# mederrata/spmf

Measured on NVIDIA B200. Metric: advi_elbo_grad_nnzK_per_s, higher is better.
Workload: dtype f32

## Files before the change

spmf_b200/csrc/spmf_hot_tile.cu:

```cuda
#include <cuda_bf16.h>
#include <cuda_runtime.h>
#include <stdint.h>
#include <stdlib.h>

#include "../../include/spmf_b200.h"
#include "spmf_record.cuh"
#include "spmf_umma_layout.cuh"
#include "spmf_umma_ptx.cuh"

namespace spmf {

__host__ __device__ __forceinline__ uint32_t core_off_g(int r, int kc, int cpr) {
  return (uint32_t)((((r >> 3) * cpr + kc) << 7) + ((r & 7) << 4));
}

template <int KP>
struct HotTile {
  static constexpr int KK = KP < 16 ? 16 : KP;
  static constexpr int CPR = KK / 8;
  static constexpr int ZCPR = CPR + 1;
  static constexpr int NZ = KK + 8;
  static constexpr int EV_TILE = 64 * KK * 2;
  static constexpr int EV_BLOCK = 2 * EV_TILE + 256;
  static constexpr int X_TILE = kTileABytes;
  static constexpr int STAGE = X_TILE + EV_BLOCK;
  static constexpr int Z_TILE = 128 * ZCPR * 16;
  static constexpr int ZCPR2 = 2 * ZCPR;
  static constexpr int W_TILE = 128 * 64 * 2;
  static constexpr bool WIDE = KK > 64;
  static constexpr bool MERGED = !WIDE;
  static constexpr int NSTAGE = WIDE ? 2 : 3;
  static constexpr int WBUF = WIDE ? 1 : 2;
  static constexpr int GHALF = WIDE ? 2 : 1;
  static constexpr int G_STRIDE = KK + 4;
  static constexpr int G_BYTES = (64 / GHALF) * G_STRIDE * 4;
  static constexpr int SMEM = NSTAGE * STAGE + 2 * Z_TILE + 2 * WBUF * W_TILE + G_BYTES + 128;
  static constexpr int ACC = MERGED ? 2 : 1;
  static constexpr int TM_S = 0, TM_DZ = 64, TM_GEV = 64 + ACC * KK, TM_GEV_STRIDE = ACC * NZ;
  static constexpr int TM_COLS = 512;
  static_assert(TM_GEV + 2 * TM_GEV_STRIDE <= 512, "tensor memory");
  static_assert(SMEM <= 227 * 1024, "shared memory");
};

__device__ __forceinline__ uint32_t pack_bf16(float a, float b) {
  __nv_bfloat162 v = __floats2bfloat162_rn(a, b);
  return *reinterpret_cast<uint32_t*>(&v);
}
__device__ __forceinline__ float bf16_lo(uint32_t p) { return __uint_as_float(p << 16); }
__device__ __forceinline__ float bf16_hi(uint32_t p) { return __uint_as_float(p & 0xffff0000u); }

template <int NC>
__device__ __forceinline__ void tmem_ld(uint32_t taddr, float* v) {
  static_assert(NC == 8 || NC == 16 || NC == 32, "tmem_ld width");
  uint32_t r[NC];
  if constexpr (NC == 32) {
    asm volatile(
        "tcgen05.ld.sync.aligned.32x32b.x32.b32 "
        "{%0, %1, %2, %3, %4, %5, %6, %7, %8, %9, %10, %11, %12, %13, %14, %15, "
        "%16, %17, %18, %19, %20, %21, %22, %23, %24, %25, %26, %27, %28, %29, %30, %31}, [%32];\n"
        : "=r"(r[0]), "=r"(r[1]), "=r"(r[2]), "=r"(r[3]), "=r"(r[4]), "=r"(r[5]), "=r"(r[6]), "=r"(r[7]),
          "=r"(r[8]), "=r"(r[9]), "=r"(r[10]), "=r"(r[11]), "=r"(r[12]), "=r"(r[13]), "=r"(r[14]), "=r"(r[15]),
          "=r"(r[16]), "=r"(r[17]), "=r"(r[18]), "=r"(r[19]), "=r"(r[20]), "=r"(r[21]), "=r"(r[22]), "=r"(r[23]),
          "=r"(r[24]), "=r"(r[25]), "=r"(r[26]), "=r"(r[27]), "=r"(r[28]), "=r"(r[29]), "=r"(r[30]), "=r"(r[31])
        : "r"(taddr));
  } else if constexpr (NC == 16) {
    asm volatile(
        "tcgen05.ld.sync.aligned.32x32b.x16.b32 "
        "{%0, %1, %2, %3, %4, %5, %6, %7, %8, %9, %10, %11, %12, %13, %14, %15}, [%16];\n"
        : "=r"(r[0]), "=r"(r[1]), "=r"(r[2]), "=r"(r[3]), "=r"(r[4]), "=r"(r[5]), "=r"(r[6]), "=r"(r[7]),
          "=r"(r[8]), "=r"(r[9]), "=r"(r[10]), "=r"(r[11]), "=r"(r[12]), "=r"(r[13]), "=r"(r[14]), "=r"(r[15])
        : "r"(taddr));
  } else {
    asm volatile("tcgen05.ld.sync.aligned.32x32b.x8.b32 {%0, %1, %2, %3, %4, %5, %6, %7}, [%8];\n"
                 : "=r"(r[0]), "=r"(r[1]), "=r"(r[2]), "=r"(r[3]), "=r"(r[4]), "=r"(r[5]), "=r"(r[6]), "=r"(r[7])
                 : "r"(taddr));
  }
  asm volatile("tcgen05.wait::ld.sync.aligned;" ::: "memory");
#pragma unroll
  for (int i = 0; i < NC; ++i) v[i] = __uint_as_float(r[i]);
}

__device__ __forceinline__ bool rate_ok_t(float lam) { return lam > 0.f && lam <= 3.402823466e38f; }

template <int KP, int SV>
__global__ void __launch_bounds__(256)
hot_ev_tiles_kernel(const float* __restrict__ EV, const float* __restrict__ PH, int D, int H,
                    unsigned char* __restrict__ EVt) {
  using T = HotTile<KP>;
  const int kc = blockIdx.x, s = blockIdx.y, nch = gridDim.x;
  const int q = s / SV, sv = s - q * SV;
  unsigned char* blk = EVt + ((size_t)s * nch + kc) * T::EV_BLOCK;
  for (int t = threadIdx.x; t < 64 * T::CPR; t += blockDim.x) {
    const int c = t / T::CPR, j = t - c * T::CPR;
    const int d = kc * 64 + c;
    float x[8];
#pragma unroll
    for (int h = 0; h < 2; ++h) {
      const int k = 8 * j + 4 * h;
      float4 v = make_float4(0.f, 0.f, 0.f, 0.f);
      if (d < H && k < KP)
        v = __ldg(reinterpret_cast<const float4*>(EV + ((size_t)q * D + d) * (SV * KP) + rec_pos(KP, SV, sv, k)));
      x[4 * h + 0] = v.x; x[4 * h + 1] = v.y; x[4 * h + 2] = v.z; x[4 * h + 3] = v.w;
    }
    uint32_t hi[4], lo[4];
#pragma unroll
    for (int p = 0; p < 4; ++p) {
      hi[p] = pack_bf16(x[2 * p], x[2 * p + 1]);
      lo[p] = pack_bf16(x[2 * p] - bf16_lo(hi[p]), x[2 * p + 1] - bf16_hi(hi[p]));
    }
    *reinterpret_cast<uint4*>(blk + core_off_g(c, j, 2 * T::CPR)) = make_uint4(hi[0], hi[1], hi[2], hi[3]);
    *reinterpret_cast<uint4*>(blk + core_off_g(c, T::CPR + j, 2 * T::CPR)) = make_uint4(lo[0], lo[1], lo[2], lo[3]);
    if (j == 0)
      reinterpret_cast<float*>(blk + 2 * T::EV_TILE)[c] = d < H ? __ldg(PH + ((size_t)q * D + d) * SV + sv) : 1.f;
  }
}

constexpr int kTileWorkThreads = 512;
constexpr int kTileThreads = kTileWorkThreads + 64;

template <int KP, int SV>
__global__ void __launch_bounds__(kTileThreads, 1)
hot_tile_kernel(const unsigned char* __restrict__ xhot, const unsigned char* __restrict__ EVt,
                const float* __restrict__ z, int nrows, int D, int H, int nch, int chunks_per_cta,
                float* __restrict__ dzacc, float* __restrict__ rowacc, float* __restrict__ GEV,
                float* __restrict__ Gphi, int* __restrict__ gflag) {
  using T = HotTile<KP>;
  constexpr int KK = T::KK, REC = SV * KP;
  extern __shared__ __align__(128) unsigned char smem_raw[];
  const uint32_t sbase = (smem_u32(smem_raw) + 127u) & ~127u;
  unsigned char* sp = smem_raw + (sbase - smem_u32(smem_raw));
  __shared__ __align__(8) unsigned long long mbar_store[T::NSTAGE + 3];
  __shared__ uint32_t tmem_slot;

  const int tid = threadIdx.x, warp = tid >> 5, lane = tid & 31;
  const int rt = tid & 127;
  const int hq = tid >> 7;
  const uint32_t lane_base = (uint32_t)((warp & 3) * 32) << 16;
  const int mt = blockIdx.x, s = blockIdx.y;
  const int q = s / SV, sv = s - q * SV;
  const int row = mt * 128 + rt;
  const int c_begin = blockIdx.z * chunks_per_cta;
  const int n = min(nch, c_begin + chunks_per_cta) - c_begin;
  if (n <= 0) return;

  const uint32_t sStage0 = sbase;
  const uint32_t sZ0 = sbase + (uint32_t)(T::NSTAGE * T::STAGE);
  const uint32_t sWb = sZ0 + 2u * (uint32_t)T::Z_TILE;
  unsigned char* const pZ0 = sp + T::NSTAGE * T::STAGE;
  unsigned char* const pWb = pZ0 + 2 * T::Z_TILE;

  uint32_t full[T::NSTAGE];
#pragma unroll
  for (int i = 0; i < T::NSTAGE; ++i) full[i] = smem_u32(&mbar_store[i]);
  const uint32_t bar_s = smem_u32(&mbar_store[T::NSTAGE]);
  const uint32_t bar_g[2] = {smem_u32(&mbar_store[T::NSTAGE + 1]), smem_u32(&mbar_store[T::NSTAGE + 2])};
  if (tid == 0) {
#pragma unroll
    for (int i = 0; i < T::NSTAGE; ++i) mbar_init(full[i], 1);
    mbar_init(bar_s, 1);
    mbar_init(bar_g[0], 2);
    mbar_init(bar_g[1], 2);
    asm volatile("fence.mbarrier_init.release.cluster;" ::: "memory");
  }
  if (warp == 3) {
    asm volatile("tcgen05.alloc.cta_group::1.sync.aligned.shared::cta.b32 [%0], %1;" ::"r"(smem_u32(&tmem_slot)),
                 "r"((uint32_t)T::TM_COLS)
                 : "memory");
    asm volatile("tcgen05.relinquish_alloc_permit.cta_group::1.sync.aligned;" ::: "memory");
  }

  const bool worker = tid < kTileWorkThreads;
  if (worker) {
    const float* zp = z + ((size_t)q * nrows + (row < nrows ? row : 0)) * REC;
#pragma unroll
    for (int j = 0; j < T::ZCPR; ++j) {
      if ((j & 3) != hq) continue;
      float zr[8];
#pragma unroll
      for (int e = 0; e < 8; ++e) zr[e] = 0.f;
      if (8 * j < KP && row < nrows) {
#pragma unroll
        for (int h = 0; h < 2; ++h) {
          if (8 * j + 4 * h < KP) {
            const float4 v = __ldg(reinterpret_cast<const float4*>(zp + rec_pos(KP, SV, sv, 8 * j + 4 * h)));
            zr[4 * h] = v.x; zr[4 * h + 1] = v.y; zr[4 * h + 2] = v.z; zr[4 * h + 3] = v.w;
          }
        }
      }
      if (8 * j == KK) zr[0] = 1.f;
      uint32_t hi[4], lo[4];
#pragma unroll
      for (int p = 0; p < 4; ++p) {
        const float a = zr[2 * p], b = zr[2 * p + 1];
        hi[p] = pack_bf16(a, b);
        lo[p] = pack_bf16(a - bf16_lo(hi[p]), b - bf16_hi(hi[p]));
      }
      *reinterpret_cast<uint4*>(pZ0 + core_off_g(rt, j, T::ZCPR2)) = make_uint4(hi[0], hi[1], hi[2], hi[3]);
      *reinterpret_cast<uint4*>(pZ0 + core_off_g(rt, T::ZCPR + j, T::ZCPR2)) = make_uint4(lo[0], lo[1], lo[2], lo[3]);
    }
  }
  asm volatile("fence.proxy.async.shared::cta;" ::: "memory");
  asm volatile("tcgen05.fence::before_thread_sync;" ::: "memory");
  __syncthreads();
  asm volatile("tcgen05.fence::after_thread_sync;" ::: "memory");
  const uint32_t tm = tmem_slot;

  const unsigned char* xsrc = xhot + ((size_t)mt * nch + c_begin) * T::X_TILE;
  const unsigned char* esrc = EVt + ((size_t)s * nch + c_begin) * T::EV_BLOCK;
  auto issue_load = [&](int i) {
    const int st = i % T::NSTAGE;
    const uint32_t dst = sStage0 + (uint32_t)(st * T::STAGE);
    mbar_expect_tx(full[st], (uint32_t)T::STAGE);
    tma_bulk_g2s(dst, xsrc + (size_t)i * T::X_TILE, T::X_TILE, full[st]);
    tma_bulk_g2s(dst + T::X_TILE, esrc + (size_t)i * T::EV_BLOCK, T::EV_BLOCK, full[st]);
  };
  auto wait_full = [&](int i) { mbar_wait(full[i % T::NSTAGE], (uint32_t)((i / T::NSTAGE) & 1)); };
  constexpr uint64_t kStageStep = (uint64_t)(T::STAGE >> 4);
  constexpr uint64_t kWStep = (uint64_t)((2 * T::W_TILE) >> 4);
  auto issue_p1 = [&](int i) {
    constexpr uint32_t ID = umma_idesc_bf16(128, 64, 0, 0);
    const uint64_t so = (uint64_t)(i % T::NSTAGE) * kStageStep;
    const uint64_t dZk[2] = {umma_desc(sZ0, 128, T::ZCPR2 * 128), umma_desc(sZ0 + T::ZCPR * 128, 128, T::ZCPR2 * 128)};
    const uint64_t dEk[2] = {umma_desc(sStage0 + T::X_TILE, 128, 2 * T::CPR * 128),
                             umma_desc(sStage0 + T::X_TILE + T::CPR * 128, 128, 2 * T::CPR * 128)};
#pragma unroll
    for (int t = 0; t < 3; ++t) {
      const uint64_t a = dZk[t == 2 ? 1 : 0], b = dEk[t == 1 ? 1 : 0] + so;
#pragma unroll
      for (int j = 0; j < KK / 16; ++j)
        umma_bf16_elect(tm + T::TM_S, a + (uint64_t)(j * 16), b + (uint64_t)(j * 16), ID, (t | j) ? 1u : 0u);
    }
    umma_commit_elect(bar_s);
  };
  float* const gst = reinterpret_cast<float*>(pWb + 2 * T::WBUF * T::W_TILE);
  auto flush_gev = [&](int i) {
    mbar_wait(bar_g[i & 1], (uint32_t)((i >> 1) & 1));
    asm volatile("tcgen05.fence::after_thread_sync;" ::: "memory");
    const uint32_t ta = tm + lane_base + T::TM_GEV + (uint32_t)((i & 1) * T::TM_GEV_STRIDE);
    const int m = (warp & 3) * 16 + lane;
    constexpr int NQD = KK >= 64 ? 4 : 2;
    constexpr int HK = KK / NQD;
    constexpr int ONES_Q = NQD == 4 ? 0 : 2;
    float g[HK], g1 = 0.f;
    if (hq < NQD) {
      tmem_ld<HK>(ta + HK * hq, g);
      if constexpr (T::MERGED) {
        float gb[HK];
        tmem_ld<HK>(ta + T::NZ + HK * hq, gb);
#pragma unroll
        for (int k = 0; k < HK; ++k) g[k] += gb[k];
      }
    }
    if (hq == ONES_Q) {
      float t8[8];
      tmem_ld<8>(ta + KK, t8);
      g1 = t8[0];
    }
    asm volatile("tcgen05.fence::before_thread_sync;" ::: "memory");
    constexpr int CPH = 64 / T::GHALF;
#pragma unroll
    for (int half = 0; half < T::GHALF; ++half) {
      if (half > 0) asm volatile("bar.sync 1, %0;" ::"n"(kTileWorkThreads) : "memory");
      const int ml = m - half * CPH;
      if (lane < 16 && ml >= 0 && ml < CPH) {
        if (hq < NQD) {
#pragma unroll
          for (int k = 0; k < HK; k += 4)
            *reinterpret_cast<float4*>(gst + ml * T::G_STRIDE + HK * hq + k) = make_float4(g[k], g[k + 1], g[k + 2], g[k + 3]);
        }
        if (hq == ONES_Q) gst[ml * T::G_STRIDE + KK] = g1;
      }
      asm volatile("bar.sync 1, %0;" ::"n"(kTileWorkThreads) : "memory");
      constexpr int TPC = KK / 4;
      constexpr int PASSES = (CPH * TPC + kTileWorkThreads - 1) / kTileWorkThreads;
#pragma unroll
      for (int ps = 0; ps < PASSES; ++ps) {
        const int idx = ps * kTileWorkThreads + tid;
        const int cl = idx / TPC, k = (idx % TPC) * 4;
        const int c = (c_begin + i) * 64 + half * CPH + cl;
        if (cl < CPH && c < H) {
          if (k < KP) {
            const float4 v = *reinterpret_cast<const float4*>(gst + cl * T::G_STRIDE + k);
            atomicAdd(reinterpret_cast<float4*>(GEV + ((size_t)q * D + c) * REC + rec_pos(KP, SV, sv, k)), v);
          }
          if ((idx % TPC) == TPC - 1) atomicAdd(Gphi + ((size_t)q * D + c) * SV + sv, gst[cl * T::G_STRIDE + KK]);
        }
      }
    }
  };

  if (warp == 17) {
    if (elect_one()) {
      issue_load(0);
      if (n > 1) issue_load(1);
      if (T::NSTAGE > 2 && n > 2) issue_load(2);
    }
    __syncwarp();
  }
  if (warp == 16) {
    wait_full(0);
    asm volatile("tcgen05.fence::after_thread_sync;" ::: "memory");
    issue_p1(0);
  }

  float xlog2 = 0.f, wmax = 0.f;
  for (int i = 0; i < n; ++i) {
    const int st = i % T::NSTAGE, wb = T::WBUF == 1 ? 0 : (i & 1), gb_ = i & 1;
    if (worker) {
    wait_full(i);
    mbar_wait(bar_s, (uint32_t)(i & 1));
    if (T::WBUF == 1 && i >= 1)
      mbar_wait(bar_g[(i - 1) & 1], (uint32_t)(((i - 1) >> 1) & 1));
    asm volatile("tcgen05.fence::after_thread_sync;" ::: "memory");

    {
      const unsigned char* xt = sp + st * T::STAGE;
      const float* ph = reinterpret_cast<const float*>(xt + T::X_TILE + 2 * T::EV_TILE) + 16 * hq;
      unsigned char* w0 = pWb + wb * 2 * T::W_TILE;
      float lam[16];
      tmem_ld<16>(tm + lane_base + T::TM_S + 16 * hq, lam);
#pragma unroll
      for (int j = 0; j < 2; ++j) {
        const uint32_t o = core_off(rt, 2 * hq + j);
        const uint4 xp = *reinterpret_cast<const uint4*>(xt + o);
        const uint32_t xw[4] = {xp.x, xp.y, xp.z, xp.w};
        const float4 p0 = *reinterpret_cast<const float4*>(ph + 8 * j);
        const float4 p1 = *reinterpret_cast<const float4*>(ph + 8 * j + 4);
        const float phv[8] = {p0.x, p0.y, p0.z, p0.w, p1.x, p1.y, p1.z, p1.w};
        float w[8];
#pragma unroll
        for (int e = 0; e < 8; ++e) {
          const float x = (e & 1) ? bf16_hi(xw[e >> 1]) : bf16_lo(xw[e >> 1]);
          const float l = fmaxf(lam[8 * j + e] + phv[e], 1e-30f);
          float lg, rc;
          asm("lg2.approx.ftz.f32 %0, %1;" : "=f"(lg) : "f"(l));
          asm("rcp.approx.ftz.f32 %0, %1;" : "=f"(rc) : "f"(l));
          w[e] = x * rc;
          wmax = fmaxf(wmax, w[e]);
          xlog2 = fmaf(x, lg, xlog2);
        }
        uint32_t hi[4], lo[4];
#pragma unroll
        for (int p = 0; p < 4; ++p) {
          hi[p] = pack_bf16(w[2 * p], w[2 * p + 1]);
          lo[p] = pack_bf16(w[2 * p] - bf16_lo(hi[p]), w[2 * p + 1] - bf16_hi(hi[p]));
        }
        *reinterpret_cast<uint4*>(w0 + o) = make_uint4(hi[0], hi[1], hi[2], hi[3]);
        *reinterpret_cast<uint4*>(w0 + T::W_TILE + o) = make_uint4(lo[0], lo[1], lo[2], lo[3]);
      }
    }
    }
    asm volatile("fence.proxy.async.shared::cta;" ::: "memory");
    asm volatile("tcgen05.fence::before_thread_sync;" ::: "memory");
    __syncthreads();

    if (warp == 17) {
      asm volatile("tcgen05.fence::after_thread_sync;" ::: "memory");
      const uint64_t wo = (uint64_t)wb * kWStep, so = (uint64_t)st * kStageStep;
      const uint64_t dWh = umma_desc(sWb, 128, 1024) + wo, dWl = umma_desc(sWb + T::W_TILE, 128, 1024) + wo;
      const uint64_t dEn = umma_desc(sStage0 + T::X_TILE, 2 * T::CPR * 128, 128) + so;
      constexpr uint64_t kEStep = (uint64_t)(2 * 2 * T::CPR * 128 / 16);
      if constexpr (T::MERGED) {
        constexpr uint32_t IDa = umma_idesc_bf16(128, 2 * KK, 0, 1), IDb = umma_idesc_bf16(128, KK, 0, 1);
#pragma unroll
        for (int j = 0; j < 4; ++j)
          umma_bf16_elect(tm + T::TM_DZ, dWh + (uint64_t)(j * 16), dEn + j * kEStep, IDa, (i | j) ? 1u : 0u);
#pragma unroll
        for (int j = 0; j < 4; ++j)
          umma_bf16_elect(tm + T::TM_DZ, dWl + (uint64_t)(j * 16), dEn + j * kEStep, IDb, 1u);
      } else {
        constexpr uint32_t ID = umma_idesc_bf16(128, KK, 0, 1);
        const uint64_t dEl = umma_desc(sStage0 + T::X_TILE + T::CPR * 128, 2 * T::CPR * 128, 128) + so;
#pragma unroll
        for (int j = 0; j < 4; ++j)
          umma_bf16_elect(tm + T::TM_DZ, dWh + (uint64_t)(j * 16), dEn + j * kEStep, ID, (i | j) ? 1u : 0u);
#pragma unroll
        for (int j = 0; j < 4; ++j)
          umma_bf16_elect(tm + T::TM_DZ, dWh + (uint64_t)(j * 16), dEl + j * kEStep, ID, 1u);
#pragma unroll
        for (int j = 0; j < 4; ++j)
          umma_bf16_elect(tm + T::TM_DZ, dWl + (uint64_t)(j * 16), dEn + j * kEStep, ID, 1u);
      }
      umma_commit_elect(bar_g[gb_]);
      if (i >= 1 && i + T::NSTAGE - 1 < n) {
        mbar_wait(bar_g[(i - 1) & 1], (uint32_t)(((i - 1) >> 1) & 1));
        if (elect_one()) issue_load(i + T::NSTAGE - 1);
        __syncwarp();
      }
    } else if (warp == 16) {
      asm volatile("tcgen05.fence::after_thread_sync;" ::: "memory");
      if (i + 1 < n) {
        wait_full(i + 1);
        asm volatile("tcgen05.fence::after_thread_sync;" ::: "memory");
        issue_p1(i + 1);
      }
      const uint64_t wo = (uint64_t)wb * kWStep;
      const uint64_t dWh = umma_desc(sWb, 1024, 128) + wo, dWl = umma_desc(sWb + T::W_TILE, 1024, 128) + wo;
      const uint64_t dZn = umma_desc(sZ0, T::ZCPR2 * 128, 128);
      constexpr uint64_t kZStep = (uint64_t)(2 * T::ZCPR2 * 128 / 16);
      const uint32_t tg = tm + T::TM_GEV + (uint32_t)(gb_ * T::TM_GEV_STRIDE);
      if constexpr (T::MERGED) {
        constexpr uint32_t IDa = umma_idesc_bf16(64, 2 * T::NZ, 1, 1), IDb = umma_idesc_bf16(64, T::NZ, 1, 1);
#pragma unroll
        for (int j = 0; j < 8; ++j)
          umma_bf16_elect(tg, dWh + (uint64_t)(j * (2048 / 16)), dZn + j * kZStep, IDa, j ? 1u : 0u);
#pragma unroll
        for (int j = 0; j < 8; ++j)
          umma_bf16_elect(tg, dWl + (uint64_t)(j * (2048 / 16)), dZn + j * kZStep, IDb, 1u);
      } else {
        constexpr uint32_t ID = umma_idesc_bf16(64, T::NZ, 1, 1);
        const uint64_t dZl = umma_desc(sZ0 + T::ZCPR * 128, T::ZCPR2 * 128, 128);
#pragma unroll
        for (int j = 0; j < 8; ++j)
          umma_bf16_elect(tg, dWh + (uint64_t)(j * (2048 / 16)), dZn + j * kZStep, ID, j ? 1u : 0u);
#pragma unroll
        for (int j = 0; j < 8; ++j)
          umma_bf16_elect(tg, dWh + (uint64_t)(j * (2048 / 16)), dZl + j * kZStep, ID, 1u);
#pragma unroll
        for (int j = 0; j < 8; ++j)
          umma_bf16_elect(tg, dWl + (uint64_t)(j * (2048 / 16)), dZn + j * kZStep, ID, 1u);
      }
      umma_commit_elect(bar_g[gb_]);
    } else if (i >= 1) {
      flush_gev(i - 1);
    }
  }
  if (worker) {
  asm volatile("bar.sync 1, %0;" ::"n"(kTileWorkThreads) : "memory");
  flush_gev(n - 1);

  {
    constexpr int QK = KK / 4;
    constexpr int LD = QK < 8 ? 8 : QK;
    float dzv[LD];
    const int col0 = QK >= 8 ? QK * hq : 8 * (hq >> 1);
    tmem_ld<LD>(tm + lane_base + T::TM_DZ + col0, dzv);
    if constexpr (T::MERGED) {
      float dzb[LD];
      tmem_ld<LD>(tm + lane_base + T::TM_DZ + KK + col0, dzb);
#pragma unroll
      for (int k = 0; k < LD; ++k) dzv[k] += dzb[k];
    }
    if (row < nrows) {
      float* dp = dzacc + ((size_t)q * nrows + row) * REC;
#pragma unroll
      for (int k = 0; k < QK; k += 4) {
        const int kk = QK * hq + k;
        const int src = (QK >= 8) ? k : 4 * (hq & 1) + k;
        if (kk < KP)
          atomicAdd(reinterpret_cast<float4*>(dp + rec_pos(KP, SV, sv, kk)),
                    make_float4(dzv[src], dzv[src + 1], dzv[src + 2], dzv[src + 3]));
      }
      atomicAdd(rowacc + ((size_t)q * nrows + row) * 4 * SV + sv, xlog2 * 0.6931471805599453f);
    }
    if (gflag && (!(wmax < 1e25f) || !(fabsf(xlog2) <= 3.402823466e38f))) atomicOr(gflag, 1);
  }
  }
  asm volatile("tcgen05.fence::before_thread_sync;" ::: "memory");
  __syncthreads();
  if (warp == 3) {
    asm volatile("tcgen05.dealloc.cta_group::1.sync.aligned.b32 %0, %1;" ::"r"(tm), "r"((uint32_t)T::TM_COLS) : "memory");
  }
}

template <int KP, int SV>
__global__ void __launch_bounds__(128)
rows_finish_kernel(const float* __restrict__ rowsum, const float* __restrict__ lgam, float inv_xi, int scale_rows,
                   int nrows, const double* __restrict__ vsum, const float* __restrict__ z,
                   float* __restrict__ dzr, float* __restrict__ rowacc, int* __restrict__ gflag) {
  constexpr int REC = SV * KP;
  static_assert(KP >= 4, "rows_finish: float4 k-vectors");
  constexpr int NCH = (REC + 127) / 128;
  const RecMap rm = rec_map(KP);
  const int row = blockIdx.x * 4 + (threadIdx.x >> 5), lane = threadIdx.x & 31, q = blockIdx.y;
  if (row >= nrows) return;
// ... 145 lines not shown
```

spmf_b200/csrc/spmf_umma.cu:

```cuda
#include <cuda_bf16.h>
#include <cuda_runtime.h>
#include <stdint.h>

#include "../../include/spmf_b200.h"
#include "spmf_umma_layout.cuh"
#include "spmf_umma_ptx.cuh"

namespace spmf {

constexpr int kGemmStages = 3;
constexpr int kGemmThreads = 128;

template <int N>
struct GemmSmem {
  static constexpr int A_BYTES = kTileABytes;
  static constexpr int B_BYTES = 3 * N * kGemmBK * 2;
  static constexpr int STAGE_BYTES = A_BYTES + B_BYTES;
  static constexpr int TOTAL = kGemmStages * STAGE_BYTES + 128;
};

template <int N>
__global__ void __launch_bounds__(kGemmThreads, 1)
umma_gemm3_kernel(const __nv_bfloat16* __restrict__ A, long long a_qstride, int M,
                  const __nv_bfloat16* __restrict__ B, long long b_qstride, float* __restrict__ C,
// ... 84 lines not shown

  const int row = m0 + tid;
  float* crow = C + (long long)row * ldc;
#pragma unroll
  for (int cb = 0; cb < N / 32; ++cb) {
    float v[32];
    tmem_ld32(tmem_acc + ((uint32_t)(warp * 32) << 16) + (uint32_t)(cb * 32), v);
    if (row < M) {
#pragma unroll
      for (int j = 0; j < 32; j += 4)
        atomicAdd(reinterpret_cast<float4*>(crow + cb * 32 + j), make_float4(v[j], v[j + 1], v[j + 2], v[j + 3]));
    }
  }
  asm volatile("tcgen05.fence::before_thread_sync;" ::: "memory");
  __syncthreads();
  if (warp == 2) {
    asm volatile("tcgen05.dealloc.cta_group::1.sync.aligned.b32 %0, %1;" ::"r"(tmem_acc), "r"((uint32_t)N) : "memory");
  }
}

__global__ void __launch_bounds__(256)
split3_transpose_kernel(const float* __restrict__ src, long long lds, long long src_qstride, int R, int Rpad,
                        int Ccols, __nv_bfloat16* __restrict__ dst, long long dst_qstride) {
  __shared__ float tile[32][33];
  const int q = blockIdx.z;
  src += (long long)q * src_qstride;
  dst += (long long)q * dst_qstride;
  const int r0 = blockIdx.x * 32, cbase = blockIdx.y * 32;
  const int tx = threadIdx.x & 31, ty = threadIdx.x >> 5;
#pragma unroll
  for (int i = 0; i < 4; ++i) {
    const int r = r0 + ty + 8 * i, c = cbase + tx;
    tile[ty + 8 * i][tx] = (r < R && c < Ccols) ? src[(long long)r * lds + c] : 0.f;
  }
  __syncthreads();
  const int c = cbase + (threadIdx.x >> 3), kq = (threadIdx.x & 7) * 4;
  if (c < Ccols && r0 + kq < Rpad) {
    __nv_bfloat16 o[3][4];
#pragma unroll
    for (int j = 0; j < 4; ++j) {
      const float x = tile[kq + j][threadIdx.x >> 3];
      const __nv_bfloat16 h = __float2bfloat16_rn(x);
      const float r1 = x - __bfloat162float(h);
      const __nv_bfloat16 m = __float2bfloat16_rn(r1);
      const float r2 = r1 - __bfloat162float(m);
      o[0][j] = h; o[1][j] = m; o[2][j] = __float2bfloat16_rn(r2);
    }
#pragma unroll
    for (int t = 0; t < 3; ++t)
      *reinterpret_cast<uint2*>(dst + tiledB_index(t, c, r0 + kq, Ccols)) = *reinterpret_cast<const uint2*>(o[t]);
  }
}

__global__ void __launch_bounds__(128, 1)
umma_probe_kernel(const unsigned char* __restrict__ a_img, int a_bytes, const unsigned char* __restrict__ b_img,
                  int b_bytes, int M, int N, int a_mn, int b_mn, int lbo_a, int sbo_a, int step_a, int lbo_b,
                  int sbo_b, int step_b, int nk, float* __restrict__ out) {
  extern __shared__ __align__(128) unsigned char smem_raw[];
  const uint32_t sbase = (smem_u32(smem_raw) + 127u) & ~127u;
  unsigned char* sp = smem_raw + (sbase - smem_u32(smem_raw));
  __shared__ __align__(8) unsigned long long mb;
  __shared__ uint32_t tslot;
  const int tid = threadIdx.x, warp = tid >> 5;
  const int a_pad = (a_bytes + 127) & ~127;
  for (int i = tid; i < a_bytes; i += 128) sp[i] = a_img[i];
  for (int i = tid; i < b_bytes; i += 128) sp[a_pad + i] = b_img[i];
  const uint32_t mbar = smem_u32(&mb);
  if (tid == 0) {
    mbar_init(mbar, 1);
    asm volatile("fence.mbarrier_init.release.cluster;" ::: "memory");
  }
  if (warp == 2) {
    asm volatile("tcgen05.alloc.cta_group::1.sync.aligned.shared::cta.b32 [%0], %1;" ::"r"(smem_u32(&tslot)), "r"(256u)
                 : "memory");
    asm volatile("tcgen05.relinquish_alloc_permit.cta_group::1.sync.aligned;" ::: "memory");
  }
  asm volatile("fence.proxy.async.shared::cta;" ::: "memory");
  asm volatile("tcgen05.fence::before_thread_sync;" ::: "memory");
  __syncthreads();
  asm volatile("tcgen05.fence::after_thread_sync;" ::: "memory");
  const uint32_t tacc = tslot;
  {
    const uint32_t taddr = tacc + ((uint32_t)(warp * 32) << 16);
    for (int c = 0; c < N; ++c)
      asm volatile("tcgen05.st.sync.aligned.32x32b.x1.b32 [%0], {%1};" ::"r"(taddr + c), "r"(0u) : "memory");
    asm volatile("tcgen05.wait::st.sync.aligned;" ::: "memory");
  }
  asm volatile("tcgen05.fence::before_thread_sync;" ::: "memory");
  __syncthreads();
  asm volatile("tcgen05.fence::after_thread_sync;" ::: "memory");
  if (tid == 0) {
    const uint32_t idesc = umma_idesc_bf16(M, N, a_mn, b_mn);
    for (int j = 0; j < nk; ++j) {
      const uint64_t ad = umma_desc(sbase + j * step_a, lbo_a, sbo_a);
      const uint64_t bd = umma_desc(sbase + a_pad + j * step_b, lbo_b, sbo_b);
      umma_bf16(tacc, ad, bd, idesc, j ? 1u : 0u);
    }
    umma_commit(mbar);
  }
  __syncwarp();
  mbar_wait(mbar, 0u);
  asm volatile("tcgen05.fence::after_thread_sync;" ::: "memory");
  for (int cb = 0; cb < N / 32; ++cb) {
    float v[32];
    tmem_ld32(tacc + ((uint32_t)(warp * 32) << 16) + (uint32_t)(cb * 32), v);
    for (int j = 0; j < 32; ++j) out[(long long)tid * N + cb * 32 + j] = v[j];
  }
  asm volatile("tcgen05.fence::before_thread_sync;" ::: "memory");
  __syncthreads();
  if (warp == 2) asm volatile("tcgen05.dealloc.cta_group::1.sync.aligned.b32 %0, %1;" ::"r"(tacc), "r"(256u) : "memory");
}

template <int N>
struct GemmAtSmem {
  static constexpr int A_BYTES = kTileABytes / 2;
  static constexpr int B_BYTES = 3 * N * kGemmBK * 2;
  static constexpr int STAGE_BYTES = A_BYTES + B_BYTES;
  static constexpr int TOTAL = kGemmStages * STAGE_BYTES + 128;
};

template <int N>
__global__ void __launch_bounds__(kGemmThreads, 1)
umma_gemm3_at_kernel(const __nv_bfloat16* __restrict__ X, int xchunks, int M,
                     const __nv_bfloat16* __restrict__ B, long long b_qstride, float* __restrict__ C,
                     long long ldc, long long c_qstride, int kchunks, int chunks_per_split, int nblocks) {
  using SM = GemmAtSmem<N>;
  extern __shared__ __align__(128) unsigned char smem_raw[];
  const uint32_t sbase = (smem_u32(smem_raw) + 127u) & ~127u;
  __shared__ __align__(8) unsigned long long mbar_store[2 * kGemmStages + 1];
  __shared__ uint32_t tmem_base_slot;

  const int tid = threadIdx.x, warp = tid >> 5, lane = tid & 31;
  const int kc = blockIdx.x;
  const int q = blockIdx.z / nblocks, nb = blockIdx.z - q * nblocks;
  const int c0 = blockIdx.y * chunks_per_split;
  const int c1 = min(kchunks, c0 + chunks_per_split);
  const int nchunks = c1 - c0;
  if (nchunks <= 0) return;
  B += (long long)q * b_qstride + (long long)nb * (N * kGemmBK);
  C += (long long)q * c_qstride + (long long)nb * N;
  const long long b_term = (long long)nblocks * N * kGemmBK;

  uint32_t full[kGemmStages], empty[kGemmStages];
#pragma unroll
  for (int i = 0; i < kGemmStages; ++i) {
    full[i] = smem_u32(&mbar_store[i]);
    empty[i] = smem_u32(&mbar_store[kGemmStages + i]);
  }
  const uint32_t done = smem_u32(&mbar_store[2 * kGemmStages]);
  if (tid == 0) {
#pragma unroll
    for (int i = 0; i < kGemmStages; ++i) { mbar_init(full[i], 1); mbar_init(empty[i], 1); }
    mbar_init(done, 1);
    asm volatile("fence.mbarrier_init.release.cluster;" ::: "memory");
  }
  if (warp == 2) {
    asm volatile("tcgen05.alloc.cta_group::1.sync.aligned.shared::cta.b32 [%0], %1;" ::"r"(smem_u32(&tmem_base_slot)),
                 "r"((uint32_t)N)
                 : "memory");
    asm volatile("tcgen05.relinquish_alloc_permit.cta_group::1.sync.aligned;" ::: "memory");
  }
  asm volatile("tcgen05.fence::before_thread_sync;" ::: "memory");
  __syncthreads();
// ... 125 lines not shown

extern "C" {

long long spmf_umma_tiled_a_elems(long long M, long long Kd) { return (M + 127) / 128 * 128 * ((Kd + 63) / 64 * 64); }
long long spmf_umma_tiled_b_elems(int N, long long Kd) { return 3LL * N * ((Kd + 63) / 64 * 64); }
long long spmf_umma_tiled_a_index(long long row, long long k, long long Kd) { return tiledA_index(row, k, Kd / kGemmBK); }

int spmf_umma_tile_a(const void* src, long long ld, int M, int Kd, void* dst, void* stream) {
  if (!src || !dst || M <= 0 || Kd <= 0 || Kd % kGemmBK) return SPMF_ERR_BAD_ARG;
  tile_a_kernel<<<148 * 4, 256, 0, (cudaStream_t)stream>>>((const __nv_bfloat16*)src, ld, M, Kd, (__nv_bfloat16*)dst);
  cudaError_t e = cudaGetLastError();
  return e == cudaSuccess ? SPMF_OK : (int)e;
}

int spmf_umma_gemm3(const void* A, long long a_qstride, int M, const void* B3, long long b_qstride, float* C,
                    long long ldc, long long c_qstride, int N, int Kd, int NQ, int splits, void* stream) {
  if (!A || !B3 || !C || M <= 0 || Kd <= 0 || NQ <= 0) return SPMF_ERR_BAD_ARG;
  if (Kd % kGemmBK || ldc % 4) return SPMF_ERR_BAD_ARG;
  if (((uintptr_t)A | (uintptr_t)B3 | (uintptr_t)C) & 15) return SPMF_ERR_BAD_ARG;
  cudaStream_t st = (cudaStream_t)stream;
  const __nv_bfloat16* a = (const __nv_bfloat16*)A;
  const __nv_bfloat16* b = (const __nv_bfloat16*)B3;
  switch (N) {
    case 32: return launch_gemm3<32>(a, a_qstride, M, b, b_qstride, C, ldc, c_qstride, Kd, NQ, splits, 1, st);
    case 64: return launch_gemm3<64>(a, a_qstride, M, b, b_qstride, C, ldc, c_qstride, Kd, NQ, splits, 1, st);
    case 128: case 256: case 512:
      return launch_gemm3<128>(a, a_qstride, M, b, b_qstride, C, ldc, c_qstride, Kd, NQ, splits, N / 128, st);
    default: return SPMF_ERR_UNSUPPORTED;
  }
}

int spmf_umma_gemm3_at(const void* X, int x_kd, int x_rows, int M, const void* B3, long long b_qstride, float* C,
                       long long ldc, long long c_qstride, int N, int NQ, int splits, void* stream) {
  if (!X || !B3 || !C || M <= 0 || x_kd <= 0 || x_rows <= 0 || NQ <= 0) return SPMF_ERR_BAD_ARG;
  if (x_kd % kGemmBK || M > x_kd || ldc % 4) return SPMF_ERR_BAD_ARG;
  if (((uintptr_t)X | (uintptr_t)B3 | (uintptr_t)C) & 15) return SPMF_ERR_BAD_ARG;
  const int Kd = (x_rows + 127) / 128 * 128;
  cudaStream_t st = (cudaStream_t)stream;
  const __nv_bfloat16* a = (const __nv_bfloat16*)X;
  const __nv_bfloat16* b = (const __nv_bfloat16*)B3;
  switch (N) {
    case 32: return launch_gemm3_at<32>(a, x_kd / kGemmBK, M, b, b_qstride, C, ldc, c_qstride, Kd, NQ, splits, 1, st);
    case 64: return launch_gemm3_at<64>(a, x_kd / kGemmBK, M, b, b_qstride, C, ldc, c_qstride, Kd, NQ, splits, 1, st);
    case 128: case 256: case 512:
      return launch_gemm3_at<128>(a, x_kd / kGemmBK, M, b, b_qstride, C, ldc, c_qstride, Kd, NQ, splits, N / 128, st);
    default: return SPMF_ERR_UNSUPPORTED;
  }
}

int spmf_umma_probe(const void* a_img, int a_bytes, const void* b_img, int b_bytes, int M, int N, int a_mn,
                    int b_mn, int lbo_a, int sbo_a, int step_a, int lbo_b, int sbo_b, int step_b, int nk,
                    float* out, void* stream) {
  if (!a_img || !b_img || !out || a_bytes <= 0 || b_bytes <= 0 || nk <= 0) return SPMF_ERR_BAD_ARG;
  if ((M != 64 && M != 128) || N % 32 || N < 32 || N > 256) return SPMF_ERR_BAD_ARG;
  const int smem = ((a_bytes + 127) & ~127) + b_bytes + 256;
  if (smem > 200 * 1024) return SPMF_ERR_BAD_ARG;
  cudaError_t e = cudaFuncSetAttribute(umma_probe_kernel, cudaFuncAttributeMaxDynamicSharedMemorySize, smem);
  if (e != cudaSuccess) return (int)e;
  umma_probe_kernel<<<1, 128, smem, (cudaStream_t)stream>>>((const unsigned char*)a_img, a_bytes,
                                                          (const unsigned char*)b_img, b_bytes, M, N, a_mn, b_mn,
                                                          lbo_a, sbo_a, step_a, lbo_b, sbo_b, step_b, nk, out);
  e = cudaGetLastError();
  return e == cudaSuccess ? SPMF_OK : (int)e;
}

int spmf_split3_transpose(const float* src, long long lds, long long src_qstride, int R, int Rpad, int Ccols,
                          void* dst3, long long dst_qstride, int NQ, void* stream) {
  if (!src || !dst3 || R <= 0 || Rpad < R || Rpad % kGemmBK || Ccols <= 0 || Ccols % 32 || NQ <= 0) return SPMF_ERR_BAD_ARG;
  dim3 grid((Rpad + 31) / 32, Ccols / 32, NQ);
  split3_transpose_kernel<<<grid, 256, 0, (cudaStream_t)stream>>>(src, lds, src_qstride, R, Rpad, Ccols,
                                                                  (__nv_bfloat16*)dst3, dst_qstride);
  cudaError_t e = cudaGetLastError();
  return e == cudaSuccess ? SPMF_OK : (int)e;
}

}
```

spmf_b200/csrc/spmf_umma_ptx.cuh:

```cuda
#pragma once
#include <cuda_runtime.h>
#include <stdint.h>

namespace spmf {

__device__ __forceinline__ uint32_t smem_u32(const void* p) {
  return (uint32_t)__cvta_generic_to_shared(p);
}

__device__ __forceinline__ uint64_t umma_desc(uint32_t saddr, uint32_t lbo, uint32_t sbo) {
  uint64_t d = 0;
  d |= (uint64_t)((saddr >> 4) & 0x3fffu);
  d |= (uint64_t)((lbo >> 4) & 0x3fffu) << 16;
  d |= (uint64_t)((sbo >> 4) & 0x3fffu) << 32;
  d |= (uint64_t)1 << 46;
  return d;
}

__host__ __device__ constexpr uint32_t umma_idesc_bf16(int M, int N, int a_mn = 0, int b_mn = 0) {
  return (1u << 4) | (1u << 7) | (1u << 10) | ((uint32_t)a_mn << 15) | ((uint32_t)b_mn << 16) |
         ((uint32_t)(N >> 3) << 17) | ((uint32_t)(M >> 4) << 24);
}

__device__ __forceinline__ void umma_bf16(uint32_t tmem_d, uint64_t adesc, uint64_t bdesc, uint32_t idesc,
                                          uint32_t accumulate) {
  asm volatile(
      "{\n\t"
      ".reg .pred p;\n\t"
      "setp.ne.b32 p, %4, 0;\n\t"
      "tcgen05.mma.cta_group::1.kind::f16 [%0], %1, %2, %3, p;\n\t"
      "}\n" ::"r"(tmem_d), "l"(adesc), "l"(bdesc), "r"(idesc), "r"(accumulate)
      : "memory");
}

__device__ __forceinline__ void umma_bf16_elect(uint32_t tmem_d, uint64_t adesc, uint64_t bdesc, uint32_t idesc,
                                                uint32_t accumulate) {
  asm volatile(
      "{\n\t"
      ".reg .pred p, e;\n\t"
      ".reg .b32 r;\n\t"
      "elect.sync r|e, 0xffffffff;\n\t"
      "setp.ne.b32 p, %4, 0;\n\t"
      "@e tcgen05.mma.cta_group::1.kind::f16 [%0], %1, %2, %3, p;\n\t"
      "}\n" ::"r"(tmem_d), "l"(adesc), "l"(bdesc), "r"(idesc), "r"(accumulate)
      : "memory");
}
__device__ __forceinline__ void umma_commit_elect(uint32_t mbar) {
  asm volatile(
      "{\n\t"
      ".reg .pred e;\n\t"
      ".reg .b32 r;\n\t"
      "elect.sync r|e, 0xffffffff;\n\t"
      "@e tcgen05.commit.cta_group::1.mbarrier::arrive::one.shared::cluster.b64 [%0];\n\t"
      "}\n" ::"r"(mbar)
      : "memory");
}
__device__ __forceinline__ bool elect_one() {
  uint32_t pred;
  asm volatile(
      "{\n\t"
      ".reg .pred e;\n\t"
      ".reg .b32 r;\n\t"
      "elect.sync r|e, 0xffffffff;\n\t"
      "selp.u32 %0, 1, 0, e;\n\t"
      "}\n"
      : "=r"(pred));
  return pred != 0;
}

__device__ __forceinline__ void umma_commit(uint32_t mbar) {
  asm volatile("tcgen05.commit.cta_group::1.mbarrier::arrive::one.shared::cluster.b64 [%0];" ::"r"(mbar)
               : "memory");
}

__device__ __forceinline__ void mbar_init(uint32_t mbar, uint32_t count) {
  asm volatile("mbarrier.init.shared::cta.b64 [%0], %1;" ::"r"(mbar), "r"(count) : "memory");
}

__device__ __forceinline__ void mbar_wait(uint32_t mbar, uint32_t parity) {
  uint32_t done;
  do {
    asm volatile(
        "{\n\t"
        ".reg .pred p;\n\t"
        "mbarrier.try_wait.parity.shared::cta.b64 p, [%1], %2;\n\t"
        "selp.u32 %0, 1, 0, p;\n\t"
        "}\n"
        : "=r"(done)
        : "r"(mbar), "r"(parity)
        : "memory");
  } while (!done);
}

__device__ __forceinline__ void tmem_ld32(uint32_t taddr, float (&v)[32]) {
  uint32_t r[32];
  asm volatile(
      "tcgen05.ld.sync.aligned.32x32b.x32.b32 "
      "{%0, %1, %2, %3, %4, %5, %6, %7, %8, %9, %10, %11, %12, %13, %14, %15, "
      "%16, %17, %18, %19, %20, %21, %22, %23, %24, %25, %26, %27, %28, %29, %30, %31}, [%32];\n"
      : "=r"(r[0]), "=r"(r[1]), "=r"(r[2]), "=r"(r[3]), "=r"(r[4]), "=r"(r[5]), "=r"(r[6]), "=r"(r[7]),
        "=r"(r[8]), "=r"(r[9]), "=r"(r[10]), "=r"(r[11]), "=r"(r[12]), "=r"(r[13]), "=r"(r[14]), "=r"(r[15]),
        "=r"(r[16]), "=r"(r[17]), "=r"(r[18]), "=r"(r[19]), "=r"(r[20]), "=r"(r[21]), "=r"(r[22]), "=r"(r[23]),
        "=r"(r[24]), "=r"(r[25]), "=r"(r[26]), "=r"(r[27]), "=r"(r[28]), "=r"(r[29]), "=r"(r[30]), "=r"(r[31])
      : "r"(taddr));
  asm volatile("tcgen05.wait::ld.sync.aligned;" ::: "memory");
#pragma unroll
  for (int i = 0; i < 32; ++i) v[i] = __uint_as_float(r[i]);
}

__device__ __forceinline__ void mbar_expect_tx(uint32_t mbar, uint32_t bytes) {
  asm volatile("mbarrier.arrive.expect_tx.shared::cta.b64 _, [%0], %1;" ::"r"(mbar), "r"(bytes) : "memory");
}
__device__ __forceinline__ void tma_bulk_g2s(uint32_t dst, const void* src, uint32_t bytes, uint32_t mbar) {
  asm volatile("cp.async.bulk.shared::cluster.global.mbarrier::complete_tx::bytes [%0], [%1], %2, [%3];" ::"r"(dst),
               "l"(src), "r"(bytes), "r"(mbar)
               : "memory");
}

}
```

Measured before the change: 255.1 billion.

## Feed UMMA A operands from tensor memory and double-buffer P1 scores for small K

For K up to 32, the z and W bf16 hi/lo tiles are also written into tensor memory, and the P1 and P2 MMAs read their A operand from TMEM instead of shared-memory descriptors. The P1 score accumulator gets a second TMEM buffer with its own mbarrier, so the MMA warp can issue P1 for chunk i+2 while workers process chunk i. The load pipeline also deepens to four stages. This aims to cut shared-memory operand traffic and the P1-to-worker serialization, at the cost of extra tcgen05.st stores and waits in the worker threads. The probe kernel gains a TMEM-A test mode.

```diff
diff --git a/spmf_b200/csrc/spmf_hot_tile.cu b/spmf_b200/csrc/spmf_hot_tile.cu
--- a/spmf_b200/csrc/spmf_hot_tile.cu
+++ b/spmf_b200/csrc/spmf_hot_tile.cu
@@ -29,7 +29,9 @@
   static constexpr int W_TILE = 128 * 64 * 2;
   static constexpr bool WIDE = KK > 64;
   static constexpr bool MERGED = !WIDE;
-  static constexpr int NSTAGE = WIDE ? 2 : 3;
+  static constexpr bool TMEM_A = KK <= 32;
+  static constexpr int SBUF = TMEM_A ? 2 : 1;
+  static constexpr int NSTAGE = WIDE ? 2 : (SBUF == 2 ? 4 : 3);
   static constexpr int WBUF = WIDE ? 1 : 2;
   static constexpr int GHALF = WIDE ? 2 : 1;
   static constexpr int G_STRIDE = KK + 4;
@@ -38,7 +40,11 @@
   static constexpr int ACC = MERGED ? 2 : 1;
   static constexpr int TM_S = 0, TM_DZ = 64, TM_GEV = 64 + ACC * KK, TM_GEV_STRIDE = ACC * NZ;
   static constexpr int TM_COLS = 512;
-  static_assert(TM_GEV + 2 * TM_GEV_STRIDE <= 512, "tensor memory");
+  static constexpr int TM_S1 = TM_GEV + 2 * TM_GEV_STRIDE;
+  static constexpr int TM_W_STRIDE = 64, TM_W = TM_COLS - 2 * TM_W_STRIDE, TM_Z = TM_W - KK;
+  static constexpr int TM_USED = TM_S1 + (TMEM_A ? 64 + KK + 2 * TM_W_STRIDE : 0);
+  static_assert(TM_USED <= TM_COLS && (!TMEM_A || TM_S1 + 64 <= TM_Z), "tensor memory");
+  static_assert(!TMEM_A || MERGED, "tensor-memory A operands: merged-term P2 only");
   static_assert(SMEM <= 227 * 1024, "shared memory");
 };
 
@@ -129,7 +135,7 @@
   extern __shared__ __align__(128) unsigned char smem_raw[];
   const uint32_t sbase = (smem_u32(smem_raw) + 127u) & ~127u;
   unsigned char* sp = smem_raw + (sbase - smem_u32(smem_raw));
-  __shared__ __align__(8) unsigned long long mbar_store[T::NSTAGE + 3];
+  __shared__ __align__(8) unsigned long long mbar_store[T::NSTAGE + 2 + T::SBUF];
   __shared__ uint32_t tmem_slot;
 
   const int tid = threadIdx.x, warp = tid >> 5, lane = tid & 31;
@@ -152,12 +158,15 @@
   uint32_t full[T::NSTAGE];
 #pragma unroll
   for (int i = 0; i < T::NSTAGE; ++i) full[i] = smem_u32(&mbar_store[i]);
-  const uint32_t bar_s = smem_u32(&mbar_store[T::NSTAGE]);
-  const uint32_t bar_g[2] = {smem_u32(&mbar_store[T::NSTAGE + 1]), smem_u32(&mbar_store[T::NSTAGE + 2])};
+  const uint32_t bar_g[2] = {smem_u32(&mbar_store[T::NSTAGE]), smem_u32(&mbar_store[T::NSTAGE + 1])};
+  uint32_t bar_s[T::SBUF];
+#pragma unroll
+  for (int b = 0; b < T::SBUF; ++b) bar_s[b] = smem_u32(&mbar_store[T::NSTAGE + 2 + b]);
   if (tid == 0) {
 #pragma unroll
     for (int i = 0; i < T::NSTAGE; ++i) mbar_init(full[i], 1);
-    mbar_init(bar_s, 1);
+#pragma unroll
+    for (int b = 0; b < T::SBUF; ++b) mbar_init(bar_s[b], 1);
     mbar_init(bar_g[0], 2);
     mbar_init(bar_g[1], 2);
     asm volatile("fence.mbarrier_init.release.cluster;" ::: "memory");
@@ -169,6 +178,11 @@
     asm volatile("tcgen05.relinquish_alloc_permit.cta_group::1.sync.aligned;" ::: "memory");
   }
 
+  asm volatile("tcgen05.fence::before_thread_sync;" ::: "memory");
+  __syncthreads();
+  asm volatile("tcgen05.fence::after_thread_sync;" ::: "memory");
+  const uint32_t tm = tmem_slot;
+
   const bool worker = tid < kTileWorkThreads;
   if (worker) {
     const float* zp = z + ((size_t)q * nrows + (row < nrows ? row : 0)) * REC;
@@ -197,13 +211,19 @@
       }
       *reinterpret_cast<uint4*>(pZ0 + core_off_g(rt, j, T::ZCPR2)) = make_uint4(hi[0], hi[1], hi[2], hi[3]);
       *reinterpret_cast<uint4*>(pZ0 + core_off_g(rt, T::ZCPR + j, T::ZCPR2)) = make_uint4(lo[0], lo[1], lo[2], lo[3]);
-    }
+      if constexpr (T::TMEM_A) {
+        if (j < T::CPR) {
+          tmem_st_x4(tm + lane_base + T::TM_Z + 4 * j, make_uint4(hi[0], hi[1], hi[2], hi[3]));
+          tmem_st_x4(tm + lane_base + T::TM_Z + KK / 2 + 4 * j, make_uint4(lo[0], lo[1], lo[2], lo[3]));
+        }
+      }
+    }
+    if constexpr (T::TMEM_A) tmem_st_wait();
   }
   asm volatile("fence.proxy.async.shared::cta;" ::: "memory");
   asm volatile("tcgen05.fence::before_thread_sync;" ::: "memory");
   __syncthreads();
   asm volatile("tcgen05.fence::after_thread_sync;" ::: "memory");
-  const uint32_t tm = tmem_slot;
 
   const unsigned char* xsrc = xhot + ((size_t)mt * nch + c_begin) * T::X_TILE;
   const unsigned char* esrc = EVt + ((size_t)s * nch + c_begin) * T::EV_BLOCK;
@@ -219,18 +239,25 @@
   constexpr uint64_t kWStep = (uint64_t)((2 * T::W_TILE) >> 4);
   auto issue_p1 = [&](int i) {
     constexpr uint32_t ID = umma_idesc_bf16(128, 64, 0, 0);
+    const uint32_t ts = tm + ((i & 1) && T::SBUF == 2 ? T::TM_S1 : T::TM_S);
     const uint64_t so = (uint64_t)(i % T::NSTAGE) * kStageStep;
     const uint64_t dZk[2] = {umma_desc(sZ0, 128, T::ZCPR2 * 128), umma_desc(sZ0 + T::ZCPR * 128, 128, T::ZCPR2 * 128)};
     const uint64_t dEk[2] = {umma_desc(sStage0 + T::X_TILE, 128, 2 * T::CPR * 128),
                              umma_desc(sStage0 + T::X_TILE + T::CPR * 128, 128, 2 * T::CPR * 128)};
 #pragma unroll
     for (int t = 0; t < 3; ++t) {
-      const uint64_t a = dZk[t == 2 ? 1 : 0], b = dEk[t == 1 ? 1 : 0] + so;
-#pragma unroll
-      for (int j = 0; j < KK / 16; ++j)
-        umma_bf16_elect(tm + T::TM_S, a + (uint64_t)(j * 16), b + (uint64_t)(j * 16), ID, (t | j) ? 1u : 0u);
-    }
-    umma_commit_elect(bar_s);
+      const uint64_t b = dEk[t == 1 ? 1 : 0] + so;
+#pragma unroll
+      for (int j = 0; j < KK / 16; ++j) {
+        if constexpr (T::TMEM_A)
+          umma_bf16_tmem_a_elect(ts, tm + T::TM_Z + (t == 2 ? KK / 2 : 0) + 8 * j, b + (uint64_t)(j * 16), ID,
+                                 (t | j) ? 1u : 0u);
+        else
+          umma_bf16_elect(ts, dZk[t == 2 ? 1 : 0] + (uint64_t)(j * 16), b + (uint64_t)(j * 16), ID,
+                          (t | j) ? 1u : 0u);
+      }
+    }
+    umma_commit_elect(bar_s[(i & 1) % T::SBUF]);
   };
   float* const gst = reinterpret_cast<float*>(pWb + 2 * T::WBUF * T::W_TILE);
   auto flush_gev = [&](int i) {
@@ -291,16 +318,21 @@
 
   if (warp == 17) {
     if (elect_one()) {
-      issue_load(0);
-      if (n > 1) issue_load(1);
-      if (T::NSTAGE > 2 && n > 2) issue_load(2);
+#pragma unroll
+      for (int k = 0; k < T::NSTAGE; ++k)
+        if (k < n) issue_load(k);
     }
     __syncwarp();
   }
   if (warp == 16) {
-    wait_full(0);
-    asm volatile("tcgen05.fence::after_thread_sync;" ::: "memory");
-    issue_p1(0);
+#pragma unroll
+    for (int k = 0; k < T::SBUF; ++k) {
+      if (k < n) {
+        wait_full(k);
+        asm volatile("tcgen05.fence::after_thread_sync;" ::: "memory");
+        issue_p1(k);
+      }
+    }
   }
 
   float xlog2 = 0.f, wmax = 0.f;
@@ -308,7 +340,7 @@
     const int st = i % T::NSTAGE, wb = T::WBUF == 1 ? 0 : (i & 1), gb_ = i & 1;
     if (worker) {
     wait_full(i);
-    mbar_wait(bar_s, (uint32_t)(i & 1));
+    mbar_wait(bar_s[(i & 1) % T::SBUF], (uint32_t)((i / T::SBUF) & 1));
     if (T::WBUF == 1 && i >= 1)
       mbar_wait(bar_g[(i - 1) & 1], (uint32_t)(((i - 1) >> 1) & 1));
     asm volatile("tcgen05.fence::after_thread_sync;" ::: "memory");
@@ -318,7 +350,7 @@
       const float* ph = reinterpret_cast<const float*>(xt + T::X_TILE + 2 * T::EV_TILE) + 16 * hq;
       unsigned char* w0 = pWb + wb * 2 * T::W_TILE;
       float lam[16];
-      tmem_ld<16>(tm + lane_base + T::TM_S + 16 * hq, lam);
+      tmem_ld<16>(tm + lane_base + ((i & 1) && T::SBUF == 2 ? T::TM_S1 : T::TM_S) + 16 * hq, lam);
 #pragma unroll
       for (int j = 0; j < 2; ++j) {
         const uint32_t o = core_off(rt, 2 * hq + j);
@@ -347,7 +379,13 @@
         }
         *reinterpret_cast<uint4*>(w0 + o) = make_uint4(hi[0], hi[1], hi[2], hi[3]);
         *reinterpret_cast<uint4*>(w0 + T::W_TILE + o) = make_uint4(lo[0], lo[1], lo[2], lo[3]);
-      }
+        if constexpr (T::TMEM_A) {
+          const uint32_t tw = tm + lane_base + T::TM_W + (uint32_t)(wb * T::TM_W_STRIDE) + 8 * hq + 4 * j;
+          tmem_st_x4(tw, make_uint4(hi[0], hi[1], hi[2], hi[3]));
+          tmem_st_x4(tw + 32, make_uint4(lo[0], lo[1], lo[2], lo[3]));
+        }
+      }
+      if constexpr (T::TMEM_A) tmem_st_wait();
     }
     }
     asm volatile("fence.proxy.async.shared::cta;" ::: "memory");
@@ -362,12 +400,21 @@
       constexpr uint64_t kEStep = (uint64_t)(2 * 2 * T::CPR * 128 / 16);
       if constexpr (T::MERGED) {
         constexpr uint32_t IDa = umma_idesc_bf16(128, 2 * KK, 0, 1), IDb = umma_idesc_bf16(128, KK, 0, 1);
-#pragma unroll
-        for (int j = 0; j < 4; ++j)
-          umma_bf16_elect(tm + T::TM_DZ, dWh + (uint64_t)(j * 16), dEn + j * kEStep, IDa, (i | j) ? 1u : 0u);
-#pragma unroll
-        for (int j = 0; j < 4; ++j)
-          umma_bf16_elect(tm + T::TM_DZ, dWl + (uint64_t)(j * 16), dEn + j * kEStep, IDb, 1u);
+        const uint32_t tWh = tm + T::TM_W + (uint32_t)(wb * T::TM_W_STRIDE), tWl = tWh + 32;
+#pragma unroll
+        for (int j = 0; j < 4; ++j) {
+          if constexpr (T::TMEM_A)
+            umma_bf16_tmem_a_elect(tm + T::TM_DZ, tWh + 8 * j, dEn + j * kEStep, IDa, (i | j) ? 1u : 0u);
+          else
+            umma_bf16_elect(tm + T::TM_DZ, dWh + (uint64_t)(j * 16), dEn + j * kEStep, IDa, (i | j) ? 1u : 0u);
+        }
+#pragma unroll
+        for (int j = 0; j < 4; ++j) {
+          if constexpr (T::TMEM_A)
+            umma_bf16_tmem_a_elect(tm + T::TM_DZ, tWl + 8 * j, dEn + j * kEStep, IDb, 1u);
+          else
+            umma_bf16_elect(tm + T::TM_DZ, dWl + (uint64_t)(j * 16), dEn + j * kEStep, IDb, 1u);
+        }
       } else {
         constexpr uint32_t ID = umma_idesc_bf16(128, KK, 0, 1);
         const uint64_t dEl = umma_desc(sStage0 + T::X_TILE + T::CPR * 128, 2 * T::CPR * 128, 128) + so;
@@ -389,7 +436,7 @@
       }
     } else if (warp == 16) {
       asm volatile("tcgen05.fence::after_thread_sync;" ::: "memory");
-      if (i + 1 < n) {
+      if (T::SBUF == 1 && i + 1 < n) {
         wait_full(i + 1);
         asm volatile("tcgen05.fence::after_thread_sync;" ::: "memory");
         issue_p1(i + 1);
@@ -421,6 +468,11 @@
           umma_bf16_elect(tg, dWl + (uint64_t)(j * (2048 / 16)), dZn + j * kZStep, ID, 1u);
       }
       umma_commit_elect(bar_g[gb_]);
+      if (T::SBUF == 2 && i + 2 < n) {
+        wait_full(i + 2);
+        asm volatile("tcgen05.fence::after_thread_sync;" ::: "memory");
+        issue_p1(i + 2);
+      }
     } else if (i >= 1) {
       flush_gev(i - 1);
     }
diff --git a/spmf_b200/csrc/spmf_umma.cu b/spmf_b200/csrc/spmf_umma.cu
--- a/spmf_b200/csrc/spmf_umma.cu
+++ b/spmf_b200/csrc/spmf_umma.cu
@@ -160,6 +160,7 @@
   }
 }
 
+constexpr int kProbeTmemA = 256;
 __global__ void __launch_bounds__(128, 1)
 umma_probe_kernel(const unsigned char* __restrict__ a_img, int a_bytes, const unsigned char* __restrict__ b_img,
                   int b_bytes, int M, int N, int a_mn, int b_mn, int lbo_a, int sbo_a, int step_a, int lbo_b,
@@ -170,8 +171,10 @@
   __shared__ __align__(8) unsigned long long mb;
   __shared__ uint32_t tslot;
   const int tid = threadIdx.x, warp = tid >> 5;
-  const int a_pad = (a_bytes + 127) & ~127;
-  for (int i = tid; i < a_bytes; i += 128) sp[i] = a_img[i];
+  const bool a_tmem = a_mn == 2;
+  const int a_pad = a_tmem ? 0 : (a_bytes + 127) & ~127;
+  if (!a_tmem)
+    for (int i = tid; i < a_bytes; i += 128) sp[i] = a_img[i];
   for (int i = tid; i < b_bytes; i += 128) sp[a_pad + i] = b_img[i];
   const uint32_t mbar = smem_u32(&mb);
   if (tid == 0) {
@@ -179,7 +182,7 @@
     asm volatile("fence.mbarrier_init.release.cluster;" ::: "memory");
   }
   if (warp == 2) {
-    asm volatile("tcgen05.alloc.cta_group::1.sync.aligned.shared::cta.b32 [%0], %1;" ::"r"(smem_u32(&tslot)), "r"(256u)
+    asm volatile("tcgen05.alloc.cta_group::1.sync.aligned.shared::cta.b32 [%0], %1;" ::"r"(smem_u32(&tslot)), "r"(512u)
                  : "memory");
     asm volatile("tcgen05.relinquish_alloc_permit.cta_group::1.sync.aligned;" ::: "memory");
   }
@@ -192,19 +195,25 @@
     const uint32_t taddr = tacc + ((uint32_t)(warp * 32) << 16);
     for (int c = 0; c < N; ++c)
       asm volatile("tcgen05.st.sync.aligned.32x32b.x1.b32 [%0], {%1};" ::"r"(taddr + c), "r"(0u) : "memory");
+    if (a_tmem) {
+      const uint4* arow = reinterpret_cast<const uint4*>(a_img + (size_t)tid * (a_bytes / 128));
+      for (int c = 0; c < a_bytes / 128 / 16; ++c) tmem_st_x4(taddr + kProbeTmemA + 4 * c, arow[c]);
+    }
     asm volatile("tcgen05.wait::st.sync.aligned;" ::: "memory");
   }
   asm volatile("tcgen05.fence::before_thread_sync;" ::: "memory");
   __syncthreads();
   asm volatile("tcgen05.fence::after_thread_sync;" ::: "memory");
-  if (tid == 0) {
-    const uint32_t idesc = umma_idesc_bf16(M, N, a_mn, b_mn);
+  if (warp == 0) {
+    const uint32_t idesc = umma_idesc_bf16(M, N, a_tmem ? 0 : a_mn, b_mn);
     for (int j = 0; j < nk; ++j) {
-      const uint64_t ad = umma_desc(sbase + j * step_a, lbo_a, sbo_a);
       const uint64_t bd = umma_desc(sbase + a_pad + j * step_b, lbo_b, sbo_b);
-      umma_bf16(tacc, ad, bd, idesc, j ? 1u : 0u);
-    }
-    umma_commit(mbar);
+      if (a_tmem)
+        umma_bf16_tmem_a_elect(tacc, tacc + kProbeTmemA + 8 * j, bd, idesc, j ? 1u : 0u);
+      else
+        umma_bf16_elect(tacc, umma_desc(sbase + j * step_a, lbo_a, sbo_a), bd, idesc, j ? 1u : 0u);
+    }
+    umma_commit_elect(mbar);
   }
   __syncwarp();
   mbar_wait(mbar, 0u);
@@ -216,7 +225,7 @@
   }
   asm volatile("tcgen05.fence::before_thread_sync;" ::: "memory");
   __syncthreads();
-  if (warp == 2) asm volatile("tcgen05.dealloc.cta_group::1.sync.aligned.b32 %0, %1;" ::"r"(tacc), "r"(256u) : "memory");
+  if (warp == 2) asm volatile("tcgen05.dealloc.cta_group::1.sync.aligned.b32 %0, %1;" ::"r"(tacc), "r"(512u) : "memory");
 }
 
 template <int N>
@@ -448,7 +457,8 @@
                     int b_mn, int lbo_a, int sbo_a, int step_a, int lbo_b, int sbo_b, int step_b, int nk,
                     float* out, void* stream) {
   if (!a_img || !b_img || !out || a_bytes <= 0 || b_bytes <= 0 || nk <= 0) return SPMF_ERR_BAD_ARG;
-  if ((M != 64 && M != 128) || N % 32 || N < 32 || N > 256) return SPMF_ERR_BAD_ARG;
+  if ((M != 64 && M != 128) || N % 32 || N < 32 || N > 256 || a_mn < 0 || a_mn > 2) return SPMF_ERR_BAD_ARG;
+  if (a_mn == 2 && (M != 128 || a_bytes != 128 * 16 * nk * 2 || 8 * nk > 512 - kProbeTmemA)) return SPMF_ERR_BAD_ARG;
   const int smem = ((a_bytes + 127) & ~127) + b_bytes + 256;
   if (smem > 200 * 1024) return SPMF_ERR_BAD_ARG;
   cudaError_t e = cudaFuncSetAttribute(umma_probe_kernel, cudaFuncAttributeMaxDynamicSharedMemorySize, smem);
diff --git a/spmf_b200/csrc/spmf_umma_ptx.cuh b/spmf_b200/csrc/spmf_umma_ptx.cuh
--- a/spmf_b200/csrc/spmf_umma_ptx.cuh
+++ b/spmf_b200/csrc/spmf_umma_ptx.cuh
@@ -22,17 +22,6 @@
          ((uint32_t)(N >> 3) << 17) | ((uint32_t)(M >> 4) << 24);
 }
 
-__device__ __forceinline__ void umma_bf16(uint32_t tmem_d, uint64_t adesc, uint64_t bdesc, uint32_t idesc,
-                                          uint32_t accumulate) {
-  asm volatile(
-      "{\n\t"
-      ".reg .pred p;\n\t"
-      "setp.ne.b32 p, %4, 0;\n\t"
-      "tcgen05.mma.cta_group::1.kind::f16 [%0], %1, %2, %3, p;\n\t"
-      "}\n" ::"r"(tmem_d), "l"(adesc), "l"(bdesc), "r"(idesc), "r"(accumulate)
-      : "memory");
-}
-
 __device__ __forceinline__ void umma_bf16_elect(uint32_t tmem_d, uint64_t adesc, uint64_t bdesc, uint32_t idesc,
                                                 uint32_t accumulate) {
   asm volatile(
@@ -45,6 +34,24 @@
       "}\n" ::"r"(tmem_d), "l"(adesc), "l"(bdesc), "r"(idesc), "r"(accumulate)
       : "memory");
 }
+__device__ __forceinline__ void umma_bf16_tmem_a_elect(uint32_t tmem_d, uint32_t tmem_a, uint64_t bdesc,
+                                                       uint32_t idesc, uint32_t accumulate) {
+  asm volatile(
+      "{\n\t"
+      ".reg .pred p, e;\n\t"
+      ".reg .b32 r;\n\t"
+      "elect.sync r|e, 0xffffffff;\n\t"
+      "setp.ne.b32 p, %4, 0;\n\t"
+      "@e tcgen05.mma.cta_group::1.kind::f16 [%0], [%1], %2, %3, p;\n\t"
+      "}\n" ::"r"(tmem_d), "r"(tmem_a), "l"(bdesc), "r"(idesc), "r"(accumulate)
+      : "memory");
+}
+__device__ __forceinline__ void tmem_st_x4(uint32_t taddr, uint4 v) {
+  asm volatile("tcgen05.st.sync.aligned.32x32b.x4.b32 [%0], {%1, %2, %3, %4};" ::"r"(taddr), "r"(v.x), "r"(v.y),
+               "r"(v.z), "r"(v.w)
+               : "memory");
+}
+__device__ __forceinline__ void tmem_st_wait() { asm volatile("tcgen05.wait::st.sync.aligned;" ::: "memory"); }
 __device__ __forceinline__ void umma_commit_elect(uint32_t mbar) {
   asm volatile(
       "{\n\t"
@@ -66,11 +73,6 @@
       "}\n"
       : "=r"(pred));
   return pred != 0;
-}
-
-__device__ __forceinline__ void umma_commit(uint32_t mbar) {
-  asm volatile("tcgen05.commit.cta_group::1.mbarrier::arrive::one.shared::cluster.b64 [%0];" ::"r"(mbar)
-               : "memory");
 }
 
 __device__ __forceinline__ void mbar_init(uint32_t mbar, uint32_t count) {
```

Measured after the change: 252.4 billion (median of 6 runs). 1.1% lower.
